# datamicroscopes/common

Measured on AMD Instinct MI355X. Metric: score_value evals/sec, higher is better.
Workload: dtype f32

## Files before the change

common_amd/csrc/kernels_niw.hip:

```cpp
#include <algorithm>
#include <cstdlib>

#include "family_math.hpp"
#include "launchers.hpp"
#include "score_block.hpp"

namespace msc {

typedef float f32x16 __attribute__((ext_vector_type(16)));


MSC_DEV size_t tri(uint32_t i, uint32_t j) { return (size_t)i * (i + 1u) / 2u + j; }
__global__ __launch_bounds__(64) void k_niw_prepare(const FeatDesc *__restrict__ feats, uint32_t f,
                                                     uint32_t K, uint32_t kpad) {
  extern __shared__ __attribute__((aligned(16))) unsigned char smem[];
  const FeatDesc fd = feats[f];
  const uint32_t d = fd.dim, k = blockIdx.x;
  const int t = threadIdx.x;
  const size_t ntri = (size_t)d * (d + 1u) / 2u;
  double *A = reinterpret_cast<double *>(smem);
  double *Li = A + ntri;
  double *mun = Li + ntri;
  double *wmu = mun + d;
  const double kappa = fd.hp[0], nu = fd.hp[1];
// ... 139 lines not shown
  for (uint64_t blk = wave_id; blk < nblocks; blk += nwaves) {
    const uint64_t rb = blk * 32 * T;
    float xr[T][16];
    int gz[T];
    bool live[T], msk[T];
#pragma unroll
    for (int t = 0; t < T; t++) {
      const uint64_t row = rb + 32 * t + r;
      live[t] = row < nrows;
      const float *xp = X + (row0 + (live[t] ? row : 0)) * d + 16 * h;
      if (d == 32) {
#pragma unroll
        for (int q = 0; q < 4; q++) {
          const float4 v = live[t] ? ld4(xp + 4 * q) : make_float4(0, 0, 0, 0);
          xr[t][4 * q] = v.x; xr[t][4 * q + 1] = v.y; xr[t][4 * q + 2] = v.z; xr[t][4 * q + 3] = v.w;
        }
      } else {
#pragma unroll
        for (int s = 0; s < 16; s++) xr[t][s] = (live[t] && (uint32_t)(16 * h + s) < d) ? xp[s] : 0.0f;
      }
      gz[t] = (LOO && live[t]) ? z[row] : -1;
      msk[t] = false;
      if (live[t] && fd.mask != nullptr)
        for (uint32_t e = 0; e < d; e++) msk[t] |= fd.mask[(row0 + row) * d + e] != 0;
    }
    float qkeep[T][4];
    for (uint32_t k = 0; k < K; k++) {
      const float *Wk = fd.niw_w + ((size_t)k * kNiwPad + r) * kNiwPad + 16 * h;
      const float *Bk = fd.niw_b + (size_t)k * 2 * kNiwPad + 16 * h;
      float w[16], mh[16], ml[16];
#pragma unroll
      for (int q = 0; q < 4; q++) {
        const float4 a = ld4(Wk + 4 * q), b = ld4(Bk + 4 * q), c = ld4(Bk + kNiwPad + 4 * q);
        w[4 * q] = a.x; w[4 * q + 1] = a.y; w[4 * q + 2] = a.z; w[4 * q + 3] = a.w;
        mh[4 * q] = b.x; mh[4 * q + 1] = b.y; mh[4 * q + 2] = b.z; mh[4 * q + 3] = b.w;
        ml[4 * q] = c.x; ml[4 * q + 1] = c.y; ml[4 * q + 2] = c.z; ml[4 * q + 3] = c.w;
      }
      const uint32_t slot = k & 3;
      const bool mine = (int)((k >> 2) & 1) == h;
#pragma unroll
      for (int t = 0; t < T; t++) {
        f32x16 acc = {0, 0, 0, 0, 0, 0, 0, 0, 0, 0, 0, 0, 0, 0, 0, 0};
#pragma unroll
        for (int s = 0; s < 16; s++)
          acc = __builtin_amdgcn_mfma_f32_32x32x2f32(w[s], (xr[t][s] - mh[s]) - ml[s], acc, 0, 0, 0);
        float qp = 0.f;
#pragma unroll
        for (int i = 0; i < 16; i++) qp = fmaf(acc[i], acc[i], qp);
        const float q = qp + __shfl_xor(qp, 32, 64);
        if (mine) {
          if (slot == 0) qkeep[t][0] = q;
          else if (slot == 1) qkeep[t][1] = q;
          else if (slot == 2) qkeep[t][2] = q;
          else qkeep[t][3] = q;
        }
      }
      if ((k & 7) == 7 || k == K - 1) {
        const uint32_t k0 = (k & ~7u) + 4 * h;
        float4 pend[T];
#pragma unroll
        for (int i = 0; i < 4; i++) {
          const uint32_t kg = k0 + i;
          const bool valid = kg <= k;
          const size_t kc = valid ? kg : 0;
          const float c0 = fd.tab[(size_t)NIW_C0 * kpad + kc], c1 = fd.tab[(size_t)NIW_C1 * kpad + kc];
#pragma unroll
          for (int t = 0; t < T; t++) {
            const float q = valid ? qkeep[t][i] : 0.f;
            float sc = fmaf(-c1, log1p_acc(q), c0);
            if (LOO && valid && gz[t] == (int)kg) {
              const float y = fminf(fd.tab[(size_t)NIW_C_LOO * kpad + kc] * q, 0.99999994f);
              sc = fmaf(fd.tab[(size_t)NIW_B_LOO * kpad + kc], log1p_acc(-y), fd.tab[(size_t)NIW_A_LOO * kpad + kc]);
            }
            if (msk[t]) sc = 0.f;
            if (i == 0) pend[t].x = sc;
            else if (i == 1) pend[t].y = sc;
            else if (i == 2) pend[t].z = sc;
            else pend[t].w = sc;
          }
        }
#pragma unroll
        for (int t = 0; t < T; t++) {
          if (!live[t] || k0 > k) continue;
          float *p = out + (rb + 32 * t + r) * ld + k0;
          if (vec_ok && k0 + 3 <= k) {
            float4 v = pend[t];
            if (ACCUM) { const float4 o = *reinterpret_cast<const float4 *>(p); v.x += o.x; v.y += o.y; v.z += o.z; v.w += o.w; }
            *reinterpret_cast<float4 *>(p) = v;
          } else {
            const float vals[4] = {pend[t].x, pend[t].y, pend[t].z, pend[t].w};
#pragma unroll
            for (int i = 0; i < 4; i++)
              if (k0 + i <= k) p[i] = ACCUM ? p[i] + vals[i] : vals[i];
          }
        }
      }
    }
  }
}

typedef double f64x4 __attribute__((ext_vector_type(4)));

MSC_DEV double shfl_xor_f64(double v, int mask) {
  const int hi = __shfl_xor(__double2hiint(v), mask, 64), lo = __shfl_xor(__double2loint(v), mask, 64);
  return __hiloint2double(hi, lo);
}

typedef unsigned int u32x2 __attribute__((ext_vector_type(2)));
MSC_DEV double xsum_rows_f64(double v) {
  u32x2 a = __builtin_amdgcn_permlane16_swap((unsigned)__double2loint(v), (unsigned)__double2loint(v), false, false);
  u32x2 b = __builtin_amdgcn_permlane16_swap((unsigned)__double2hiint(v), (unsigned)__double2hiint(v), false, false);
  const double s = __hiloint2double((int)b[0], (int)a[0]) + __hiloint2double((int)b[1], (int)a[1]);
  a = __builtin_amdgcn_permlane32_swap((unsigned)__double2loint(s), (unsigned)__double2loint(s), false, false);
  b = __builtin_amdgcn_permlane32_swap((unsigned)__double2hiint(s), (unsigned)__double2hiint(s), false, false);
  return __hiloint2double((int)b[0], (int)a[0]) + __hiloint2double((int)b[1], (int)a[1]);
}

template <int ROWS>
MSC_DEV double pair_rows_f64(double x, double y) {
  u32x2 lo, hi;
  if (ROWS == 16) {
    lo = __builtin_amdgcn_permlane16_swap((unsigned)__double2loint(x), (unsigned)__double2loint(y), false, false);
    hi = __builtin_amdgcn_permlane16_swap((unsigned)__double2hiint(x), (unsigned)__double2hiint(y), false, false);
  } else {
    lo = __builtin_amdgcn_permlane32_swap((unsigned)__double2loint(x), (unsigned)__double2loint(y), false, false);
    hi = __builtin_amdgcn_permlane32_swap((unsigned)__double2hiint(x), (unsigned)__double2hiint(y), false, false);
  }
  return __hiloint2double((int)hi[0], (int)lo[0]) + __hiloint2double((int)hi[1], (int)lo[1]);
}

MSC_DEV double log_ge1_f64(double u) {
  int hi = __double2hiint(u);
  int e = (hi >> 20) - 1023;
  double m = __hiloint2double((hi & 0x000fffff) | 0x3ff00000, __double2loint(u));
  if (m > 1.4142135623730951) {
    m *= 0.5;
    e += 1;
  }
  const double den = m + 1.0;
  double y = __builtin_amdgcn_rcp(den);
  y = y * fma(-den, y, 2.0);
  y = y * fma(-den, y, 2.0);
  const double sq = (m - 1.0) * y, s2 = sq * sq;
  double p = 1.0 / 15.0;
  p = fma(p, s2, 1.0 / 13.0);
  p = fma(p, s2, 1.0 / 11.0);
  p = fma(p, s2, 1.0 / 9.0);
  p = fma(p, s2, 1.0 / 7.0);
  p = fma(p, s2, 1.0 / 5.0);
  p = fma(p, s2, 1.0 / 3.0);
  p = fma(p, s2, 1.0);
  return fma((double)e, 0.69314718055994530942, 2.0 * sq * p);
}
MSC_DEV double niw_score_from_q(double c0, double c1, double q) { return c0 - c1 * log_ge1_f64(1.0 + q); }

template <int JB, bool LOO, bool ACCUM, bool FULL = false>
MSC_DEV void niw64_finish_batch(const FeatDesc &fd, uint32_t k, int kk, int c, uint64_t rb, const double (&qkeep)[JB][4],
                                const int (&gz)[JB], const bool (&msk)[JB], const bool (&live)[JB],
                                double *__restrict__ qown, float *__restrict__ out, uint64_t ld, bool vec_ok) {
  const uint32_t k0 = (k & ~15u) + 4 * kk;
  float4 pend[JB];
#pragma unroll
  for (int i = 0; i < 4; i++) {
    const uint32_t kg = k0 + i;
    const bool valid = FULL || kg <= k;
    const double *c64 = fd.niw_c64 + (size_t)(valid ? kg : 0) * 8;
    const double c0 = c64[0], c1 = c64[1];
#pragma unroll
    for (int jb = 0; jb < JB; jb++) {
      const double q = valid ? qkeep[jb][i] : 0.0;
      double sc = niw_score_from_q(c0, c1, q);
      if (LOO && valid && gz[jb] == (int)kg) {
        qown[rb + 16 * jb + c] = q;
        sc = 0.0;
      }
      if (msk[jb]) sc = 0.0;
      const float scf = (float)sc;
      if (i == 0) pend[jb].x = scf;
      else if (i == 1) pend[jb].y = scf;
      else if (i == 2) pend[jb].z = scf;
      else pend[jb].w = scf;
    }
  }
#pragma unroll
  for (int jb = 0; jb < JB; jb++) {
    if (!live[jb] || (!FULL && k0 > k)) continue;
    float *p = out + (rb + 16 * jb + c) * ld + k0;
    if (vec_ok && (FULL || k0 + 3 <= k)) {
      float4 v = pend[jb];
      if (ACCUM) { const float4 o = *reinterpret_cast<const float4 *>(p); v.x += o.x; v.y += o.y; v.z += o.z; v.w += o.w; }
      *reinterpret_cast<float4 *>(p) = v;
    } else {
      const float vals[4] = {pend[jb].x, pend[jb].y, pend[jb].z, pend[jb].w};
#pragma unroll
      for (int i = 0; i < 4; i++)
        if (k0 + i <= k) p[i] = ACCUM ? p[i] + vals[i] : vals[i];
    }
  }
}

template <int NB, int JB, bool LOO, bool ACCUM>
__global__ __launch_bounds__(256) void k_score_niw64(const FeatDesc *__restrict__ feats, uint32_t f,
                                                      uint32_t K, uint32_t kpad, uint64_t row0,
                                                      uint64_t nrows, const int32_t *__restrict__ z,
                                                      double *__restrict__ qown, float *__restrict__ out, uint64_t ld) {
  constexpr int NS = 4 * NB;
  constexpr int NCH = NB * (NB + 1) / 2;
  const FeatDesc fd = feats[f];
  const uint32_t d = fd.dim;
  const int lane = threadIdx.x & 63, c = lane & 15, kk = lane >> 4;
  const uint64_t nblocks = (nrows + 16 * JB - 1) / (16 * JB);
  const uint64_t wave_id = (uint64_t)blockIdx.x * 4 + (threadIdx.x >> 6);
  const uint64_t nwaves = (uint64_t)gridDim.x * 4;
  const float *X = reinterpret_cast<const float *>(fd.col);
  const bool vec_ok = ((ld & 3) == 0) && ((reinterpret_cast<uintptr_t>(out) & 15) == 0);
  for (uint64_t blk = wave_id; blk < nblocks; blk += nwaves) {
    const uint64_t rb = blk * 16 * JB;
    float xf[JB][NS];
    int gz[JB];
    bool live[JB], msk[JB];
#pragma unroll
    for (int jb = 0; jb < JB; jb++) {
      const uint64_t row = rb + 16 * jb + c;
      live[jb] = row < nrows;
      const float *xp = X + (row0 + (live[jb] ? row : 0)) * d + kk;
#pragma unroll
      for (int s = 0; s < NS; s++) xf[jb][s] = (live[jb] && (uint32_t)(4 * s + kk) < d) ? xp[4 * s] : 0.0f;
      gz[jb] = (LOO && live[jb]) ? z[row] : -1;
      msk[jb] = false;
      if (live[jb] && fd.mask != nullptr)
        for (uint32_t e = 0; e < d; e++) msk[jb] |= fd.mask[(row0 + row) * d + e] != 0;
    }
    double qkeep[JB][4];
    for (uint32_t k = 0; k < K; k++) {
      const double *Wk = fd.niw_w64 + (size_t)k * (NCH * 256) + lane * 4;
      const double *Bk = fd.niw_mu64 + (size_t)k * (NB * 256) + lane * 4;
      double qp[JB];
#pragma unroll
      for (int jb = 0; jb < JB; jb++) qp[jb] = 0.0;
      constexpr bool PIPE = NB > 2;
      double2 n01 = {0.0, 0.0}, n23 = {0.0, 0.0};
      if (PIPE) {
        n01 = *reinterpret_cast<const double2 *>(Wk);
        n23 = *reinterpret_cast<const double2 *>(Wk + 2);
      }
#pragma unroll
      for (int b = 0; b < NB; b++) {
        const double2 b01 = *reinterpret_cast<const double2 *>(Bk + b * 256), b23 = *reinterpret_cast<const double2 *>(Bk + b * 256 + 2);
        f64x4 acc[JB];
#pragma unroll
        for (int jb = 0; jb < JB; jb++) acc[jb] = f64x4{-b01.x, -b01.y, -b23.x, -b23.y};
#pragma unroll
        for (int s4 = 0; s4 <= b; s4++) {
          constexpr int kLast = NCH - 1;
          const int ch = b * (b + 1) / 2 + s4;
          const double *wc = Wk + ch * 256;
          double2 a01, a23;
          if (PIPE) {
            a01 = n01;
            a23 = n23;
            if (ch < kLast) {
              n01 = *reinterpret_cast<const double2 *>(wc + 256);
              n23 = *reinterpret_cast<const double2 *>(wc + 256 + 2);
            }
          } else {
            a01 = *reinterpret_cast<const double2 *>(wc);
            a23 = *reinterpret_cast<const double2 *>(wc + 2);
          }
          const double a[4] = {a01.x, a01.y, a23.x, a23.y};
#pragma unroll
          for (int e = 0; e < 4; e++) {
#pragma unroll
            for (int jb = 0; jb < JB; jb++) {
              float xv = xf[jb][4 * s4 + e];
              if (NB > 2) asm volatile("" : "+v"(xv));
              acc[jb] = __builtin_amdgcn_mfma_f64_16x16x4f64(a[e], (double)xv, acc[jb], 0, 0, 0);
            }
          }
          if (PIPE) __builtin_amdgcn_sched_barrier(0);
        }
#pragma unroll
        for (int jb = 0; jb < JB; jb++)
#pragma unroll
          for (int i = 0; i < 4; i++) qp[jb] = fma(acc[jb][i], acc[jb][i], qp[jb]);
      }
      const uint32_t slot = k & 3;
      const bool mine = (int)((k >> 2) & 3) == kk;
#pragma unroll
      for (int jb = 0; jb < JB; jb++) {
        const double q = xsum_rows_f64(qp[jb]);
        if (mine) {
          if (slot == 0) qkeep[jb][0] = q;
          else if (slot == 1) qkeep[jb][1] = q;
          else if (slot == 2) qkeep[jb][2] = q;
          else qkeep[jb][3] = q;
        }
      }
      if ((k & 15) == 15 || k == K - 1) {
        const uint32_t k0 = (k & ~15u) + 4 * kk;
        float4 pend[JB];
#pragma unroll
        for (int i = 0; i < 4; i++) {
          const uint32_t kg = k0 + i;
          const bool valid = kg <= k;
          const double *c64 = fd.niw_c64 + (size_t)(valid ? kg : 0) * 8;
          const double c0 = c64[0], c1 = c64[1];
#pragma unroll
          for (int jb = 0; jb < JB; jb++) {
            const double q = valid ? qkeep[jb][i] : 0.0;
            double sc = niw_score_from_q(c0, c1, q);
            if (LOO && valid && gz[jb] == (int)kg) {
              qown[rb + 16 * jb + c] = q;
              sc = 0.0;
            }
            if (msk[jb]) sc = 0.0;
            const float scf = (float)sc;
            if (i == 0) pend[jb].x = scf;
            else if (i == 1) pend[jb].y = scf;
            else if (i == 2) pend[jb].z = scf;
            else pend[jb].w = scf;
          }
        }
#pragma unroll
        for (int jb = 0; jb < JB; jb++) {
          if (!live[jb] || k0 > k) continue;
          float *p = out + (rb + 16 * jb + c) * ld + k0;
          if (vec_ok && k0 + 3 <= k) {
            float4 v = pend[jb];
            if (ACCUM) { const float4 o = *reinterpret_cast<const float4 *>(p); v.x += o.x; v.y += o.y; v.z += o.z; v.w += o.w; }
            *reinterpret_cast<float4 *>(p) = v;
          } else {
            const float vals[4] = {pend[jb].x, pend[jb].y, pend[jb].z, pend[jb].w};
#pragma unroll
            for (int i = 0; i < 4; i++)
              if (k0 + i <= k) p[i] = ACCUM ? p[i] + vals[i] : vals[i];
          }
        }
      }
    }
  }
}

template <int NB, bool LOO, bool ACCUM>
__global__ __launch_bounds__(256, 2) void k_score_niw64_lag(const FeatDesc *__restrict__ feats, uint32_t f,
                                                             uint32_t K, uint32_t kpad, uint64_t row0,
                                                             uint64_t nrows, const int32_t *z,
                                                             double *__restrict__ qown, float *__restrict__ out, uint64_t ld) {
  static_assert(NB == 1 || NB == 2, "dim <= 32");
  constexpr int JB = 4, NS = 4 * NB, NCH = NB * (NB + 1) / 2;
  const FeatDesc fd = feats[f];
  const uint32_t d = fd.dim;
  const int lane = threadIdx.x & 63, c = lane & 15, kk = lane >> 4;
  const uint64_t nblocks = (nrows + 16 * JB - 1) / (16 * JB);
  const uint64_t wave_id = (uint64_t)blockIdx.x * 4 + (threadIdx.x >> 6);
  const uint64_t nwaves = (uint64_t)gridDim.x * 4;
  const float *X = reinterpret_cast<const float *>(fd.col);
  const bool vec_ok = ((ld & 3) == 0) && ((reinterpret_cast<uintptr_t>(out) & 15) == 0);
  typedef uint32_t u32x4v __attribute__((ext_vector_type(4)));
  const __amdgpu_buffer_rsrc_t Wb = __builtin_amdgcn_make_buffer_rsrc(const_cast<double *>(fd.niw_w64), 0, 0x7fffffff, 0x00020000);
  const __amdgpu_buffer_rsrc_t Bb = __builtin_amdgcn_make_buffer_rsrc(const_cast<double *>(fd.niw_mu64), 0, 0x7fffffff, 0x00020000);
  const uint32_t lane_off = lane * 32;
  const uint32_t Kfull = K & ~15u;
  auto group_at = [&](uint32_t t) -> uint32_t {
    const uint32_t g = t < Kfull ? (t & ~15u) + 4 * (t & 3) + ((t >> 2) & 3) : t;
    return g < K ? g : K - 1;
  };
  for (uint64_t blk = wave_id; blk < nblocks; blk += nwaves) {
    const uint64_t rb = blk * 16 * JB;
    float xn[JB][NS];
    int gz[JB];
    bool live[JB], msk[JB];
#pragma unroll
    for (int jb = 0; jb < JB; jb++) {
      const uint64_t row = rb + 16 * jb + c;
      live[jb] = row < nrows;
      const float *xp = X + (row0 + (live[jb] ? row : 0)) * d;
#pragma unroll
      for (int s = 0; s < NS; s++) {
        const bool has = live[jb] && (uint32_t)(4 * s + kk) < d;
        const float v = xp[has ? 4 * s + kk : 0];
        xn[jb][s] = has ? -v : 0.0f;
      }
      gz[jb] = (LOO && live[jb]) ? z[row] : -1;
      msk[jb] = false;
      if (live[jb] && fd.mask != nullptr)
        for (uint32_t e = 0; e < d; e++) msk[jb] |= fd.mask[(row0 + row) * d + e] != 0;
    }
    double qkeep[JB][4];
    double2 w0[2], w1[2], w2[2], m0[2], m1[2];
    auto load2 = [&](double2 (&o)[2], __amdgpu_buffer_rsrc_t buf, uint32_t byte) {
      const u32x4v lo = __builtin_amdgcn_raw_buffer_load_b128(buf, lane_off, byte, 0);
      const u32x4v hi = __builtin_amdgcn_raw_buffer_load_b128(buf, lane_off + 16, byte, 0);
      o[0] = double2{__hiloint2double((int)lo[1], (int)lo[0]), __hiloint2double((int)lo[3], (int)lo[2])};
      o[1] = double2{__hiloint2double((int)hi[1], (int)hi[0]), __hiloint2double((int)hi[3], (int)hi[2])};
    };
    auto chunk = [&](f64x4 (&acc)[JB], const double2 (&w)[2], int s4, const double2 (*m)[2]) {
      const double a[4] = {w[0].x, w[0].y, w[1].x, w[1].y};
#pragma unroll
      for (int e = 0; e < 4; e++)
#pragma unroll
        for (int jb = 0; jb < JB; jb++) {
          const f64x4 from = (m != nullptr && e == 0) ? f64x4{(*m)[0].x, (*m)[0].y, (*m)[1].x, (*m)[1].y} : acc[jb];
          acc[jb] = __builtin_amdgcn_mfma_f64_16x16x4f64(a[e], (double)xn[jb][4 * s4 + e], from, 0, 0, 0);
        }
    };
    auto squares = [](double (&qp)[JB], const f64x4 (&acc)[JB], bool fresh) {
#pragma unroll
      for (int jb = 0; jb < JB; jb++)
#pragma unroll
        for (int i = 0; i < 4; i++) qp[jb] = (fresh && i == 0) ? acc[jb][i] * acc[jb][i] : fma(acc[jb][i], acc[jb][i], qp[jb]);
    };
    f64x4 accA[JB], accB[JB];
    double qp[JB], held[JB], half[JB];
    if constexpr (NB == 2) {
      const uint32_t g0 = group_at(0), g1 = group_at(1);
      load2(w0, Wb, g0 * (NCH * 2048u));
      load2(m0, Bb, g0 * (NB * 2048u));
      load2(w1, Wb, g0 * (NCH * 2048u) + 2048);
      load2(w2, Wb, g0 * (NCH * 2048u) + 4096);
      load2(m1, Bb, g0 * (NB * 2048u) + 2048);
      chunk(accA, w0, 0, &m0);
      load2(w0, Wb, g1 * (NCH * 2048u));
      load2(m0, Bb, g1 * (NB * 2048u));
    } else {
      const uint32_t g0 = group_at(0), g1 = group_at(1), g2 = group_at(2);
      load2(w0, Wb, g0 * 2048u);
      load2(m0, Bb, g0 * 2048u);
      load2(w1, Wb, g1 * 2048u);
      load2(m1, Bb, g1 * 2048u);
      chunk(accA, w0, 0, &m0);
      load2(w0, Wb, g2 * 2048u);
      load2(m0, Bb, g2 * 2048u);
    }
    for (uint32_t t4 = 0; t4 < K; t4 += 4) {
      const bool tail = t4 >= Kfull;
      const bool mine = (int)((t4 >> 2) & 3) == kk;
#pragma unroll
      for (int i = 0; i < 4; i++) {
        if constexpr (NB == 2) {
          const uint32_t gn = group_at(t4 + i + 1), gn2 = group_at(t4 + i + 2);
          chunk(accB, w1, 0, &m1);
          chunk(accB, w2, 1, nullptr);
          squares(qp, accA, true);
          load2(w1, Wb, gn * (NCH * 2048u) + 2048);
          load2(w2, Wb, gn * (NCH * 2048u) + 4096);
          load2(m1, Bb, gn * (NB * 2048u) + 2048);
          __builtin_amdgcn_sched_barrier(0);
          chunk(accA, w0, 0, &m0);
          squares(qp, accB, false);
          load2(w0, Wb, gn2 * (NCH * 2048u));
          load2(m0, Bb, gn2 * (NB * 2048u));
          __builtin_amdgcn_sched_barrier(0);
        } else {
          const uint32_t gn3 = group_at(t4 + i + 3);
          if ((i & 1) == 0) {
            chunk(accB, w1, 0, &m1);
            squares(qp, accA, true);
            load2(w1, Wb, gn3 * 2048u);
            load2(m1, Bb, gn3 * 2048u);
          } else {
            chunk(accA, w0, 0, &m0);
            squares(qp, accB, true);
            load2(w0, Wb, gn3 * 2048u);
            load2(m0, Bb, gn3 * 2048u);
          }
          __builtin_amdgcn_sched_barrier(0);
        }
        if (!tail) {
          if (i == 0 || i == 2) {
#pragma unroll
            for (int jb = 0; jb < JB; jb++) held[jb] = qp[jb];
          } else {
#pragma unroll
            for (int jb = 0; jb < JB; jb++) {
              const double pr = pair_rows_f64<16>(held[jb], qp[jb]);
              if (i == 1) half[jb] = pr;
              else {
                const double q = pair_rows_f64<32>(half[jb], pr);
                qkeep[jb][0] = qkeep[jb][1];
                qkeep[jb][1] = qkeep[jb][2];
                qkeep[jb][2] = qkeep[jb][3];
                qkeep[jb][3] = q;
              }
            }
          }
        } else {
#pragma unroll
          for (int jb = 0; jb < JB; jb++) {
            const double q = xsum_rows_f64(qp[jb]);
            qkeep[jb][i] = mine ? q : qkeep[jb][i];
          }
        }
      }
      const uint32_t kl = t4 + 3 < K ? t4 + 3 : K - 1;
      if ((kl & 15) == 15) niw64_finish_batch<JB, LOO, ACCUM, true>(fd, kl, kk, c, rb, qkeep, gz, msk, live, qown, out, ld, vec_ok);
      else if (kl == K - 1) niw64_finish_batch<JB, LOO, ACCUM>(fd, kl, kk, c, rb, qkeep, gz, msk, live, qown, out, ld, vec_ok);
    }
  }
}

template <int NB, bool LOO, bool ACCUM>
__global__ __launch_bounds__(256, NB <= 5 ? 3 : 2) void k_score_niw64_wide(const FeatDesc *__restrict__ feats, uint32_t f,
                                                           uint32_t K, uint32_t kpad, uint64_t row0,
                                                           uint64_t nrows, const int32_t *z,
                                                           double *__restrict__ qown, float *__restrict__ out, uint64_t ld) {
  static_assert(NB > 2 && NB <= 8, "32 < dim <= 128");
  constexpr int JB = 2, NS = 4 * NB, NCH = NB * (NB + 1) / 2;
  const FeatDesc fd = feats[f];
  const uint32_t d = fd.dim;
  const int lane = threadIdx.x & 63, c = lane & 15, kk = lane >> 4;
  const uint64_t nblocks = (nrows + 16 * JB - 1) / (16 * JB);
  const uint64_t wave_id = (uint64_t)blockIdx.x * 4 + (threadIdx.x >> 6);
  const uint64_t nwaves = (uint64_t)gridDim.x * 4;
  const float *X = reinterpret_cast<const float *>(fd.col);
  const bool vec_ok = ((ld & 3) == 0) && ((reinterpret_cast<uintptr_t>(out) & 15) == 0);
  typedef uint32_t u32x4v __attribute__((ext_vector_type(4)));
  const __amdgpu_buffer_rsrc_t Wb = __builtin_amdgcn_make_buffer_rsrc(const_cast<double *>(fd.niw_w64), 0, 0x7fffffff, 0x00020000);
  const __amdgpu_buffer_rsrc_t Bb = __builtin_amdgcn_make_buffer_rsrc(const_cast<double *>(fd.niw_mu64), 0, 0x7fffffff, 0x00020000);
  const uint32_t lane_off = lane * 32;
  const uint32_t Kfull = K & ~15u;
  auto group_at = [&](uint32_t t) -> uint32_t {
    const uint32_t g = t < Kfull ? (t & ~15u) + 4 * (t & 3) + ((t >> 2) & 3) : t;
    return g < K ? g : K - 1;
  };
  auto load2 = [&](double2 (&o)[2], __amdgpu_buffer_rsrc_t buf, uint32_t byte) {
    const u32x4v lo = __builtin_amdgcn_raw_buffer_load_b128(buf, lane_off, byte, 0);
    const u32x4v hi = __builtin_amdgcn_raw_buffer_load_b128(buf, lane_off + 16, byte, 0);
    o[0] = double2{__hiloint2double((int)lo[1], (int)lo[0]), __hiloint2double((int)lo[3], (int)lo[2])};
    o[1] = double2{__hiloint2double((int)hi[1], (int)hi[0]), __hiloint2double((int)hi[3], (int)hi[2])};
  };
  for (uint64_t blk = wave_id; blk < nblocks; blk += nwaves) {
    const uint64_t rb = blk * 16 * JB;
    float xn[JB][NS];
    int gz[JB];
    bool live[JB], msk[JB];
#pragma unroll
    for (int jb = 0; jb < JB; jb++) {
      const uint64_t row = rb + 16 * jb + c;
      live[jb] = row < nrows;
      const float *xp = X + (row0 + (live[jb] ? row : 0)) * d;
#pragma unroll
      for (int s = 0; s < NS; s++) {
        const bool has = live[jb] && (uint32_t)(4 * s + kk) < d;
        const float v = xp[has ? 4 * s + kk : 0];
        xn[jb][s] = has ? -v : 0.0f;
      }
      gz[jb] = (LOO && live[jb]) ? z[row] : -1;
      msk[jb] = false;
      if (live[jb] && fd.mask != nullptr)
        for (uint32_t e = 0; e < d; e++) msk[jb] |= fd.mask[(row0 + row) * d + e] != 0;
    }
    double qkeep[JB][4], held[JB], half[JB];
    double2 nxt[2];
    load2(nxt, Wb, group_at(0) * (NCH * 2048u));
    const uint32_t Kt = (K + 3u) & ~3u;
    for (uint32_t t = 0; t < Kt; t++) {
      const uint32_t g = group_at(t), gn = group_at(t + 1);
      const int i = (int)(t & 3u);
      const bool tail = t >= Kfull;
      double qp[JB];
#pragma unroll
      for (int jb = 0; jb < JB; jb++) qp[jb] = 0.0;
#pragma unroll
      for (int b = 0; b < NB; b++) {
        double2 m[2];
        load2(m, Bb, g * (NB * 2048u) + b * 2048u);
        const f64x4 mv = {m[0].x, m[0].y, m[1].x, m[1].y};
        f64x4 acc[JB];
#pragma unroll
        for (int s4 = 0; s4 <= b; s4++) {
          constexpr int kLast = NCH - 1;
          const int ch = b * (b + 1) / 2 + s4;
          const double a[4] = {nxt[0].x, nxt[0].y, nxt[1].x, nxt[1].y};
          if (ch < kLast) load2(nxt, Wb, g * (NCH * 2048u) + (ch + 1) * 2048u);
          else load2(nxt, Wb, gn * (NCH * 2048u));
#pragma unroll
          for (int e = 0; e < 4; e++)
#pragma unroll
            for (int jb = 0; jb < JB; jb++) {
              float xv = xn[jb][4 * s4 + e];
              asm volatile("" : "+v"(xv));
              acc[jb] = __builtin_amdgcn_mfma_f64_16x16x4f64(a[e], (double)xv, (s4 == 0 && e == 0) ? mv : acc[jb], 0, 0, 0);
            }
          __builtin_amdgcn_sched_barrier(0);
        }
#pragma unroll
        for (int jb = 0; jb < JB; jb++)
#pragma unroll
          for (int q = 0; q < 4; q++) qp[jb] = fma(acc[jb][q], acc[jb][q], qp[jb]);
      }
      if (!tail) {
        if (i == 0 || i == 2) {
#pragma unroll
          for (int jb = 0; jb < JB; jb++) held[jb] = qp[jb];
        } else {
#pragma unroll
          for (int jb = 0; jb < JB; jb++) {
            const double pr = pair_rows_f64<16>(held[jb], qp[jb]);
            if (i == 1) half[jb] = pr;
            else {
              const double q = pair_rows_f64<32>(half[jb], pr);
              qkeep[jb][0] = qkeep[jb][1];
              qkeep[jb][1] = qkeep[jb][2];
              qkeep[jb][2] = qkeep[jb][3];
              qkeep[jb][3] = q;
            }
          }
        }
      } else {
        const bool mine = (int)((t >> 2) & 3) == kk;
#pragma unroll
        for (int jb = 0; jb < JB; jb++) {
          const double q = xsum_rows_f64(qp[jb]);
          if (mine) {
            if (i == 0) qkeep[jb][0] = q;
            else if (i == 1) qkeep[jb][1] = q;
            else if (i == 2) qkeep[jb][2] = q;
            else qkeep[jb][3] = q;
          }
        }
      }
      if (i == 3) {
        const uint32_t kl = t < K ? t : K - 1;
        if ((kl & 15) == 15) niw64_finish_batch<JB, LOO, ACCUM, true>(fd, kl, kk, c, rb, qkeep, gz, msk, live, qown, out, ld, vec_ok);
        else if (kl == K - 1) niw64_finish_batch<JB, LOO, ACCUM>(fd, kl, kk, c, rb, qkeep, gz, msk, live, qown, out, ld, vec_ok);
      }
    }
  }
}

MSC_DEV double bcast_f64(double v, int lane) {
  return __hiloint2double(__builtin_amdgcn_readlane(__double2hiint(v), lane), __builtin_amdgcn_readlane(__double2loint(v), lane));
}
template <int D>
__global__ __launch_bounds__(256) void k_score_niw_small(const FeatDesc *__restrict__ feats, uint32_t f, uint32_t K,
                                                          uint32_t kpad, uint64_t row0, uint64_t nrows,
                                                          const int32_t *__restrict__ z, double *__restrict__ qown,
                                                          float *__restrict__ out, uint64_t ld, int accum) {
  const FeatDesc fd = feats[f];
  const int lane = threadIdx.x & 63;
  const uint32_t k = blockIdx.y * 64 + lane;
  const bool has_k = k < K;
  const size_t kc = has_k ? k : 0;
  double w[D * (D + 1) / 2], nb[D];
#pragma unroll
  for (int i = 0; i < D; i++) {
#pragma unroll
    for (int j = 0; j <= i; j++) w[i * (i + 1) / 2 + j] = fd.niw_w64[kc * niw_w_stream(D) + niw_w_index(i, j)];
    nb[i] = -fd.niw_mu64[kc * niw_b_stream(D) + niw_b_index(i)];
// ... 78 lines not shown
                                                           uint64_t row0, uint64_t nrows,
                                                           const int32_t *__restrict__ z, uint32_t *__restrict__ scratch) {
  extern __shared__ uint32_t hist[];
  const FeatDesc fd = feats[f];
  const bool lds = K <= kBucketLdsGroups;
  if (lds) {
    for (uint32_t k = threadIdx.x; k < K; k += 256) hist[k] = 0u;
    __syncthreads();
  }
  const uint64_t per = (nrows + gridDim.x - 1) / gridDim.x, lo = (uint64_t)blockIdx.x * per;
  const uint64_t hi = lo + per < nrows ? lo + per : nrows;
  for (uint64_t n = lo + threadIdx.x; n < hi; n += 256)
    if (niw_row_counts(fd, K, row0 + n, z[n])) atomicAdd(lds ? &hist[z[n]] : &scratch[K + 1 + z[n]], 1u);
  if (lds) {
    __syncthreads();
    for (uint32_t k = threadIdx.x; k < K; k += 256)
      if (hist[k]) atomicAdd(&scratch[K + 1 + k], hist[k]);
  }
}
__global__ __launch_bounds__(1024) void k_niw_bucket_scan(uint32_t K, uint32_t *__restrict__ scratch) {
  __shared__ uint32_t part[1024];
  const uint32_t per = (K + 1023) / 1024, lo = threadIdx.x * per, hi = lo + per < K ? lo + per : K;
  uint32_t s = 0;
  for (uint32_t k = lo; k < hi; k++) s += scratch[K + 1 + k];
  part[threadIdx.x] = s;
  __syncthreads();
  for (int off = 1; off < 1024; off <<= 1) {
    const uint32_t v = threadIdx.x >= (uint32_t)off ? part[threadIdx.x - off] : 0u;
    __syncthreads();
    part[threadIdx.x] += v;
    __syncthreads();
  }
  uint32_t run = threadIdx.x ? part[threadIdx.x - 1] : 0u;
  for (uint32_t k = lo; k < hi; k++) {
    const uint32_t c = scratch[K + 1 + k];
    scratch[k] = run;
    scratch[K + 1 + k] = 0u;
    run += c;
  }
  if (threadIdx.x == 1023) scratch[K] = part[1023];
}
__global__ __launch_bounds__(256) void k_niw_bucket_scatter(const FeatDesc *__restrict__ feats, uint32_t f, uint32_t K,
                                                             uint64_t row0, uint64_t nrows,
                                                             const int32_t *__restrict__ z, uint32_t *__restrict__ scratch) {
  extern __shared__ uint32_t sh[];
  const FeatDesc fd = feats[f];
  uint32_t *idx = scratch + 2 * (size_t)K + 1;
  const uint64_t per = (nrows + gridDim.x - 1) / gridDim.x, lo = (uint64_t)blockIdx.x * per;
  const uint64_t hi = lo + per < nrows ? lo + per : nrows;
  if (K > kBucketLdsGroups) {
    for (uint64_t n = lo + threadIdx.x; n < hi; n += 256) {
      const int g = z[n];
      if (niw_row_counts(fd, K, row0 + n, g)) idx[scratch[g] + atomicAdd(&scratch[K + 1 + g], 1u)] = (uint32_t)n;
    }
    return;
  }
  uint32_t *cnt = sh, *base = sh + K;
  for (uint32_t k = threadIdx.x; k < K; k += 256) cnt[k] = 0u;
  __syncthreads();
  for (uint64_t n = lo + threadIdx.x; n < hi; n += 256)
    if (niw_row_counts(fd, K, row0 + n, z[n])) atomicAdd(&cnt[z[n]], 1u);
  __syncthreads();
  for (uint32_t k = threadIdx.x; k < K; k += 256) {
    base[k] = cnt[k] ? scratch[k] + atomicAdd(&scratch[K + 1 + k], cnt[k]) : 0u;
    cnt[k] = 0u;
  }
  __syncthreads();
  for (uint64_t n = lo + threadIdx.x; n < hi; n += 256) {
    const int g = z[n];
    if (niw_row_counts(fd, K, row0 + n, g)) idx[base[g] + atomicAdd(&cnt[g], 1u)] = (uint32_t)n;
  }
}
__global__ __launch_bounds__(256) void k_niw_group_sums(const FeatDesc *__restrict__ feats, uint32_t f, uint32_t K,
                                                         uint64_t row0, const uint32_t *__restrict__ scratch, int sign) {
  __shared__ float xs[4][2][32];
  __shared__ double red[4][17][64];
  const FeatDesc fd = feats[f];
  const uint32_t d = fd.dim, k = blockIdx.x;
  const uint32_t nt = (d + 31u) / 32u, ti = blockIdx.z / nt, tj = blockIdx.z % nt;
  const int lane = threadIdx.x & 63, wave = threadIdx.x >> 6;
  const uint32_t i = (uint32_t)lane >> 1, half = (uint32_t)lane & 1u;
  const uint32_t beg = scratch[k], end = scratch[k + 1];
  const uint32_t *idx = scratch + 2 * (size_t)K + 1;
  const float *X = reinterpret_cast<const float *>(fd.col);
  double sxx[16], sx = 0.0;
#pragma unroll
  for (int j = 0; j < 16; j++) sxx[j] = 0.0;
  for (uint32_t p = beg + blockIdx.y * 4 + wave; p < end; p += gridDim.y * 4) {
    const float *x = X + (row0 + idx[p]) * d;
    const uint32_t e = (uint32_t)(lane & 31), src = 32u * (lane < 32 ? ti : tj) + e;
    xs[wave][lane >> 5][e] = src < d ? x[src] : 0.f;
    const double xi = (double)xs[wave][0][i];
    if (half == 0) sx += xi;
#pragma unroll
    for (int j = 0; j < 16; j++) sxx[j] = fma(xi, (double)xs[wave][1][half * 16 + j], sxx[j]);
  }
#pragma unroll
  for (int j = 0; j < 16; j++) red[wave][j][lane] = sxx[j];
  red[wave][16][lane] = sx;
  __syncthreads();
  if (end == beg) return;
  const size_t stride = d + (size_t)d * d;
  double *dst = fd.acc_f64 + (size_t)k * stride;
  for (uint32_t e = threadIdx.x; e < 17 * 64; e += 256) {
    const uint32_t j = e >> 6, l = e & 63, ii = 32u * ti + (l >> 1), hh = l & 1u;
    const double v = red[0][j][l] + red[1][j][l] + red[2][j][l] + red[3][j][l];
    if (ii >= d) continue;
    if (j == 16) {
      if (tj == 0 && hh == 0 && v != 0.0) atomicAdd(&dst[ii], (double)sign * v);
    } else {
      const uint32_t col = 32u * tj + hh * 16 + j;
      if (col < d && v != 0.0) atomicAdd(&dst[d + (size_t)ii * d + col], (double)sign * v);
    }
  }
  if (blockIdx.y == 0 && blockIdx.z == 0 && threadIdx.x == 0)
    atomicAdd(reinterpret_cast<unsigned long long *>(&fd.acc_i64[k]), (unsigned long long)((long long)sign * (long long)(end - beg)));
}

__global__ __launch_bounds__(256) void k_niw_commit(const FeatDesc *__restrict__ feats, uint32_t f,
                                                     uint32_t K, uint32_t kpad, int to_raw) {
  const FeatDesc fd = feats[f];
  const size_t stride = fd.dim + (size_t)fd.dim * fd.dim, total = (size_t)K * stride;
  const size_t i = (size_t)blockIdx.x * 256 + threadIdx.x;
  if (i < total) {
    if (to_raw) fd.raw_f32[i] = (float)fd.acc_f64[i];
    else fd.acc_f64[i] = (double)fd.raw_f32[i];
  }
  if (i < kpad) {
    if (to_raw) fd.raw_u32[i] = (uint32_t)fd.acc_i64[i];
    else fd.acc_i64[i] = fd.raw_u32[i];
  }
}

int launch_niw_prepare(hipStream_t stream, const FeatDesc *feats_dev, uint32_t f, uint32_t dim, uint32_t K,
                       uint32_t kpad) {
  const size_t lds = sizeof(double) * ((size_t)dim * (dim + 1) + 2 * (size_t)dim);
  static unsigned long long attr_devices = 0;
  if (lds > 64u * 1024u && first_use_on_device(attr_devices))
    (void)hipFuncSetAttribute(reinterpret_cast<const void *>(k_niw_prepare), hipFuncAttributeMaxDynamicSharedMemorySize, 160 * 1024);
  hipLaunchKernelGGL(k_niw_prepare, dim3(K + 1), dim3(64), lds, stream, feats_dev, f, K, kpad);
  return hipGetLastError() == hipSuccess ? 0 : -1;
}

int launch_niw_score_data(hipStream_t stream, const FeatDesc *feats_dev, uint32_t f, uint32_t K,
                          uint32_t kpad, float *out) {
  hipLaunchKernelGGL(k_niw_score_data, dim3((K + 255) / 256), dim3(256), 0, stream, feats_dev, f, K, kpad, out);
  return hipGetLastError() == hipSuccess ? 0 : -1;
}

template <int NB, bool LOO, bool ACCUM>
static void launch_niw64_nb(hipStream_t stream, const dim3 grid, const FeatDesc *feats_dev, uint32_t f, uint32_t K, uint32_t kpad,
                            uint64_t row0, uint64_t nrows, const int32_t *z, double *qown, float *out, uint64_t ld) {
  if constexpr (NB <= 2) {
    if ((uint64_t)K * 6144u < 0x7fffffffull) {
      hipLaunchKernelGGL((k_score_niw64_lag<NB, LOO, ACCUM>), (note_kernel(0, "k_score_niw64_lag<%d, %s, %s>", NB, tf(LOO), tf(ACCUM)), grid), dim3(256), 0, stream, feats_dev, f, K, kpad, row0, nrows, z, qown, out, ld);
      return;
    }
  }
  if constexpr (NB > 2) {
    if ((uint64_t)K * (NB * (NB + 1) / 2) * 2048u < 0x7fffffffull)
      hipLaunchKernelGGL((k_score_niw64_wide<NB, LOO, ACCUM>), (note_kernel(0, "k_score_niw64_wide<%d, %s, %s>", NB, tf(LOO), tf(ACCUM)), dim3(grid.x * 2)), dim3(256), 0, stream, feats_dev, f, K, kpad, row0, nrows, z, qown, out, ld);
    else
      hipLaunchKernelGGL((k_score_niw64<NB, 2, LOO, ACCUM>), (note_kernel(0, "k_score_niw64<%d, 2, %s, %s>", NB, tf(LOO), tf(ACCUM)), dim3(grid.x * 2)), dim3(256), 0, stream, feats_dev, f, K, kpad, row0, nrows, z, qown, out, ld);
  } else
    hipLaunchKernelGGL((k_score_niw64<NB, 4, LOO, ACCUM>), (note_kernel(0, "k_score_niw64<%d, 4, %s, %s>", NB, tf(LOO), tf(ACCUM)), grid), dim3(256), 0, stream, feats_dev, f, K, kpad, row0, nrows, z, qown, out, ld);
}
template <bool LOO, bool ACCUM>
static void launch_niw_score_t(hipStream_t stream, int num_cus, bool f32_fast, uint32_t dim, const FeatDesc *feats_dev,
                               uint32_t f, uint32_t K, uint32_t kpad, uint64_t row0, uint64_t nrows,
                               const int32_t *z, double *qown, float *out, uint64_t ld) {
  constexpr int kRowsPerWave = 64;
  const uint64_t nblocks = (nrows + kRowsPerWave - 1) / kRowsPerWave;
  uint64_t gx = (nblocks + 3) / 4;
  const uint64_t cap = (uint64_t)num_cus * 8;
  if (gx > cap) gx = cap;
  const dim3 grid((unsigned)(gx ? gx : 1)), block(256);
  if (f32_fast && dim <= (uint32_t)kNiwPad)
    hipLaunchKernelGGL((k_score_niw<2, LOO, ACCUM>), (note_kernel(0, "k_score_niw<2, %s, %s>", tf(LOO), tf(ACCUM)), grid), block, 0, stream, feats_dev, f, K, kpad, row0, nrows, z, out, ld);
  else {
    switch (niw_blocks(dim)) {
      case 1: launch_niw64_nb<1, LOO, ACCUM>(stream, grid, feats_dev, f, K, kpad, row0, nrows, z, qown, out, ld); break;
      case 2: launch_niw64_nb<2, LOO, ACCUM>(stream, grid, feats_dev, f, K, kpad, row0, nrows, z, qown, out, ld); break;
      case 3: launch_niw64_nb<3, LOO, ACCUM>(stream, grid, feats_dev, f, K, kpad, row0, nrows, z, qown, out, ld); break;
      case 4: launch_niw64_nb<4, LOO, ACCUM>(stream, grid, feats_dev, f, K, kpad, row0, nrows, z, qown, out, ld); break;
      case 5: launch_niw64_nb<5, LOO, ACCUM>(stream, grid, feats_dev, f, K, kpad, row0, nrows, z, qown, out, ld); break;
      case 6: launch_niw64_nb<6, LOO, ACCUM>(stream, grid, feats_dev, f, K, kpad, row0, nrows, z, qown, out, ld); break;
      case 7: launch_niw64_nb<7, LOO, ACCUM>(stream, grid, feats_dev, f, K, kpad, row0, nrows, z, qown, out, ld); break;
      default: launch_niw64_nb<8, LOO, ACCUM>(stream, grid, feats_dev, f, K, kpad, row0, nrows, z, qown, out, ld); break;
    }
    if (LOO)
      hipLaunchKernelGGL(k_niw_loo_patch, dim3((unsigned)((nrows + 255) / 256)), dim3(256), 0, stream, feats_dev, f, K, row0,
                         nrows, z, qown, out, ld);
  }
}

template <int D>
static void launch_niw_small(hipStream_t stream, int num_cus, const FeatDesc *feats_dev, uint32_t f, uint32_t K, uint32_t kpad,
                             uint64_t row0, uint64_t nrows, const int32_t *z, double *qown, float *out, uint64_t ld, bool accum) {
  const uint32_t ktiles = (K + 63) / 64;
  uint64_t gx = ((nrows + 63) / 64 + 3) / 4;
  const uint64_t cap = std::max<uint64_t>(1, (uint64_t)num_cus * 8 / ktiles);
  if (gx > cap) gx = cap;
  hipLaunchKernelGGL(k_score_niw_small<D>, dim3((unsigned)(gx ? gx : 1), ktiles), dim3(256), 0, stream, feats_dev, f, K, kpad,
                     row0, nrows, z, qown, out, ld, accum ? 1 : 0);
  if (z != nullptr)
    hipLaunchKernelGGL(k_niw_loo_patch, dim3((unsigned)((nrows + 255) / 256)), dim3(256), 0, stream, feats_dev, f, K, row0,
                       nrows, z, qown, out, ld);
}

int launch_niw_score(hipStream_t stream, int num_cus, const FeatDesc *feats_dev, uint32_t f, uint32_t dim, uint32_t K,
                     uint32_t kpad, uint64_t row0, uint64_t nrows, const int32_t *z, bool accum, bool f32_fast,
                     double *qown, float *out, uint64_t ld) {
  if (!f32_fast && dim >= 1 && dim <= 8 && nrows > 0) {
    switch (dim) {
      case 1: launch_niw_small<1>(stream, num_cus, feats_dev, f, K, kpad, row0, nrows, z, qown, out, ld, accum); break;
      case 2: launch_niw_small<2>(stream, num_cus, feats_dev, f, K, kpad, row0, nrows, z, qown, out, ld, accum); break;
      case 3: launch_niw_small<3>(stream, num_cus, feats_dev, f, K, kpad, row0, nrows, z, qown, out, ld, accum); break;
      case 4: launch_niw_small<4>(stream, num_cus, feats_dev, f, K, kpad, row0, nrows, z, qown, out, ld, accum); break;
      case 5: launch_niw_small<5>(stream, num_cus, feats_dev, f, K, kpad, row0, nrows, z, qown, out, ld, accum); break;
      case 6: launch_niw_small<6>(stream, num_cus, feats_dev, f, K, kpad, row0, nrows, z, qown, out, ld, accum); break;
      case 7: launch_niw_small<7>(stream, num_cus, feats_dev, f, K, kpad, row0, nrows, z, qown, out, ld, accum); break;
      default: launch_niw_small<8>(stream, num_cus, feats_dev, f, K, kpad, row0, nrows, z, qown, out, ld, accum); break;
    }
    return hipGetLastError() == hipSuccess ? 0 : -1;
  }
  if (z && accum) launch_niw_score_t<true, true>(stream, num_cus, f32_fast, dim, feats_dev, f, K, kpad, row0, nrows, z, qown, out, ld);
  else if (z) launch_niw_score_t<true, false>(stream, num_cus, f32_fast, dim, feats_dev, f, K, kpad, row0, nrows, z, qown, out, ld);
  else if (accum) launch_niw_score_t<false, true>(stream, num_cus, f32_fast, dim, feats_dev, f, K, kpad, row0, nrows, z, qown, out, ld);
  else launch_niw_score_t<false, false>(stream, num_cus, f32_fast, dim, feats_dev, f, K, kpad, row0, nrows, z, qown, out, ld);
  return hipGetLastError() == hipSuccess ? 0 : -1;
}

template <int D>
__global__ __launch_bounds__(1024) void k_niw_accumulate_small(const FeatDesc *__restrict__ feats, uint32_t f, uint32_t K,
                                                                uint64_t row0, uint64_t nrows, const int32_t *__restrict__ z,
                                                                int sign) {
  extern __shared__ __attribute__((aligned(16))) unsigned char smem[];
  constexpr uint32_t kStride = D + D * D;
  const FeatDesc fd = feats[f];
  double *sums = reinterpret_cast<double *>(smem);
  uint32_t *cnt = reinterpret_cast<uint32_t *>(sums + (size_t)K * kStride);
  for (uint32_t i = threadIdx.x; i < K * kStride; i += blockDim.x) sums[i] = 0.0;
  for (uint32_t i = threadIdx.x; i < K; i += blockDim.x) cnt[i] = 0u;
  __syncthreads();
  const uint64_t per = (nrows + gridDim.x - 1) / gridDim.x;
  const uint64_t lo = (uint64_t)blockIdx.x * per, hi = lo + per < nrows ? lo + per : nrows;
  const float *X = reinterpret_cast<const float *>(fd.col);
  for (uint64_t n = lo + threadIdx.x; n < hi; n += blockDim.x) {
    const int g = z[n];
    const uint64_t row = row0 + n;
    if (!niw_row_counts(fd, K, row, g)) continue;
    double x[D];
#pragma unroll
    for (int j = 0; j < D; j++) x[j] = (double)X[row * D + j];
    double *dst = sums + (size_t)g * kStride;
    atomicAdd(&cnt[g], 1u);
#pragma unroll
    for (int i = 0; i < D; i++) {
      atomicAdd(&dst[i], x[i]);
#pragma unroll
      for (int j = 0; j < D; j++) atomicAdd(&dst[D + i * D + j], x[i] * x[j]);
    }
  }
  __syncthreads();
  for (uint32_t i = threadIdx.x; i < K * kStride; i += blockDim.x)
    if (sums[i] != 0.0) atomicAdd(&fd.acc_f64[i], (double)sign * sums[i]);
  for (uint32_t i = threadIdx.x; i < K; i += blockDim.x)
    if (cnt[i]) atomicAdd(reinterpret_cast<unsigned long long *>(&fd.acc_i64[i]), (unsigned long long)((long long)sign * (long long)cnt[i]));
}
template <int D>
static void launch_niw_accumulate_small(hipStream_t stream, int num_cus, const FeatDesc *feats_dev, uint32_t f, uint32_t K,
                                        uint64_t row0, uint64_t nrows, const int32_t *z, int sign, size_t lds) {
  static unsigned long long attr_devices = 0;
  if (first_use_on_device(attr_devices))
    (void)hipFuncSetAttribute(reinterpret_cast<const void *>(k_niw_accumulate_small<D>),
                              hipFuncAttributeMaxDynamicSharedMemorySize, 160 * 1024);
  uint64_t blocks = (nrows + 4095) / 4096;
  if (blocks < (uint64_t)num_cus) blocks = (nrows + 1023) / 1024;
  if (blocks > (uint64_t)num_cus * 2) blocks = (uint64_t)num_cus * 2;
  hipLaunchKernelGGL(k_niw_accumulate_small<D>, dim3((unsigned)(blocks ? blocks : 1)), dim3(1024), lds, stream, feats_dev, f, K,
                     row0, nrows, z, sign);
}

int launch_niw_accumulate(hipStream_t stream, int num_cus, const FeatDesc *feats_dev, uint32_t f, uint32_t K,
                          uint64_t row0, uint64_t nrows, const int32_t *z, int sign, uint32_t *scratch_dev, uint32_t dim) {
  if (nrows == 0) return 0;
  const size_t small_lds = (size_t)K * ((dim + (size_t)dim * dim) * sizeof(double) + sizeof(uint32_t));
  if (dim >= 1 && dim <= 8 && small_lds <= 96u * 1024u) {
    switch (dim) {
      case 1: launch_niw_accumulate_small<1>(stream, num_cus, feats_dev, f, K, row0, nrows, z, sign, small_lds); break;
      case 2: launch_niw_accumulate_small<2>(stream, num_cus, feats_dev, f, K, row0, nrows, z, sign, small_lds); break;
      case 3: launch_niw_accumulate_small<3>(stream, num_cus, feats_dev, f, K, row0, nrows, z, sign, small_lds); break;
      case 4: launch_niw_accumulate_small<4>(stream, num_cus, feats_dev, f, K, row0, nrows, z, sign, small_lds); break;
      case 5: launch_niw_accumulate_small<5>(stream, num_cus, feats_dev, f, K, row0, nrows, z, sign, small_lds); break;
      case 6: launch_niw_accumulate_small<6>(stream, num_cus, feats_dev, f, K, row0, nrows, z, sign, small_lds); break;
      case 7: launch_niw_accumulate_small<7>(stream, num_cus, feats_dev, f, K, row0, nrows, z, sign, small_lds); break;
      default: launch_niw_accumulate_small<8>(stream, num_cus, feats_dev, f, K, row0, nrows, z, sign, small_lds); break;
    }
    return hipGetLastError() == hipSuccess ? 0 : -1;
  }
  if (hipMemsetAsync(scratch_dev, 0, sizeof(uint32_t) * (2 * (size_t)K + 1), stream) != hipSuccess) return -1;
  uint64_t gx = (nrows + 255) / 256;
  const uint64_t cap = (uint64_t)num_cus * 8;
  if (gx > cap) gx = cap;
  const size_t lds1 = K <= kBucketLdsGroups ? sizeof(uint32_t) * K : 0, lds2 = 2 * lds1;
  hipLaunchKernelGGL(k_niw_bucket_count, dim3((unsigned)gx), dim3(256), lds1, stream, feats_dev, f, K, row0, nrows, z, scratch_dev);
  hipLaunchKernelGGL(k_niw_bucket_scan, dim3(1), dim3(1024), 0, stream, K, scratch_dev);
// ... 21 lines not shown
```

Measured before the change: 1478 billion.

## Finish NIW scores per group inside lag kernel loop with buffer stores

Restructures the lagged NIW64 scoring kernel so each 4-cluster group's score is computed and written immediately after its reduction, rather than keeping a shifting qkeep buffer and calling a batched finish routine every 16 clusters. Score constants and outputs go through buffer resources, and the log coefficients are pinned in scalar registers. Inputs are widened to double once at load time rather than inside each MFMA. This cuts register pressure and spreads the transcendental and store work across the MFMA pipeline, at the cost of more, smaller scalar stores. A new launch guard keeps 32-bit buffer offsets valid.

Result: no change. 1473 billion, median of 6 (-0.3%).

```diff
diff --git a/common_amd/csrc/kernels_niw.hip b/common_amd/csrc/kernels_niw.hip
--- a/common_amd/csrc/kernels_niw.hip
+++ b/common_amd/csrc/kernels_niw.hip
@@ -315,7 +315,35 @@
   p = fma(p, s2, 1.0);
   return fma((double)e, 0.69314718055994530942, 2.0 * sq * p);
 }
+#define MSC_LOG_GE1_COEFS \
+  {1.0 / 15.0, 1.0 / 13.0, 1.0 / 11.0, 1.0 / 9.0, 1.0 / 7.0, 1.0 / 5.0, 1.0 / 3.0, 1.4142135623730951, 0.69314718055994530942}
+MSC_DEV double log_ge1_f64(double u, const double (&k)[9], int bias) {
+  int hi = __double2hiint(u);
+  int e = (hi >> 20) - bias;
+  double m = __hiloint2double((hi & 0x000fffff) | 0x3ff00000, __double2loint(u));
+  if (m > k[7]) {
+    m *= 0.5;
+    e += 1;
+  }
+  const double den = m + 1.0;
+  double y = __builtin_amdgcn_rcp(den);
+  y = y * fma(-den, y, 2.0);
+  y = y * fma(-den, y, 2.0);
+  const double sq = (m - 1.0) * y, s2 = sq * sq;
+  double p = k[0];
+  p = fma(p, s2, k[1]);
+  p = fma(p, s2, k[2]);
+  p = fma(p, s2, k[3]);
+  p = fma(p, s2, k[4]);
+  p = fma(p, s2, k[5]);
+  p = fma(p, s2, k[6]);
+  p = fma(p, s2, 1.0);
+  return fma((double)e, k[8], 2.0 * sq * p);
+}
 MSC_DEV double niw_score_from_q(double c0, double c1, double q) { return c0 - c1 * log_ge1_f64(1.0 + q); }
+MSC_DEV double niw_score_from_q(double c0, double c1, double q, const double (&k)[9], int bias) {
+  return c0 - c1 * log_ge1_f64(1.0 + q, k, bias);
+}
 
 template <int JB, bool LOO, bool ACCUM, bool FULL = false>
 MSC_DEV void niw64_finish_batch(const FeatDesc &fd, uint32_t k, int kk, int c, uint64_t rb, const double (&qkeep)[JB][4],
@@ -518,11 +546,12 @@
   const uint64_t wave_id = (uint64_t)blockIdx.x * 4 + (threadIdx.x >> 6);
   const uint64_t nwaves = (uint64_t)gridDim.x * 4;
   const float *X = reinterpret_cast<const float *>(fd.col);
-  const bool vec_ok = ((ld & 3) == 0) && ((reinterpret_cast<uintptr_t>(out) & 15) == 0);
   typedef uint32_t u32x4v __attribute__((ext_vector_type(4)));
   const __amdgpu_buffer_rsrc_t Wb = __builtin_amdgcn_make_buffer_rsrc(const_cast<double *>(fd.niw_w64), 0, 0x7fffffff, 0x00020000);
   const __amdgpu_buffer_rsrc_t Bb = __builtin_amdgcn_make_buffer_rsrc(const_cast<double *>(fd.niw_mu64), 0, 0x7fffffff, 0x00020000);
+  const __amdgpu_buffer_rsrc_t Cb = __builtin_amdgcn_make_buffer_rsrc(fd.niw_c64, 0, 0x7fffffff, 0x00020000);
   const uint32_t lane_off = lane * 32;
+  const uint32_t row_off = (uint32_t)c * (uint32_t)ld * 4u + 16u * kk;
   const uint32_t Kfull = K & ~15u;
   auto group_at = [&](uint32_t t) -> uint32_t {
     const uint32_t g = t < Kfull ? (t & ~15u) + 4 * (t & 3) + ((t >> 2) & 3) : t;
@@ -530,26 +559,32 @@
   };
   for (uint64_t blk = wave_id; blk < nblocks; blk += nwaves) {
     const uint64_t rb = blk * 16 * JB;
-    float xn[JB][NS];
+    const __amdgpu_buffer_rsrc_t Ob = __builtin_amdgcn_make_buffer_rsrc(out + rb * ld, 0, 0x7fffffff, 0x00020000);
+    const __amdgpu_buffer_rsrc_t Qb = __builtin_amdgcn_make_buffer_rsrc(LOO ? qown + rb : qown, 0, 0x7fffffff, 0x00020000);
+    double xn[JB][NS];
     int gz[JB];
     bool live[JB], msk[JB];
+    uint32_t cr = (uint32_t)c;
+    asm volatile("" : "+v"(cr));
 #pragma unroll
     for (int jb = 0; jb < JB; jb++) {
-      const uint64_t row = rb + 16 * jb + c;
+      const uint64_t row = rb + 16 * jb + cr;
       live[jb] = row < nrows;
-      const float *xp = X + (row0 + (live[jb] ? row : 0)) * d;
-#pragma unroll
-      for (int s = 0; s < NS; s++) {
-        const bool has = live[jb] && (uint32_t)(4 * s + kk) < d;
-        const float v = xp[has ? 4 * s + kk : 0];
-        xn[jb][s] = has ? -v : 0.0f;
-      }
       gz[jb] = (LOO && live[jb]) ? z[row] : -1;
       msk[jb] = false;
       if (live[jb] && fd.mask != nullptr)
         for (uint32_t e = 0; e < d; e++) msk[jb] |= fd.mask[(row0 + row) * d + e] != 0;
     }
-    double qkeep[JB][4];
+#pragma unroll
+    for (int jb = 0; jb < JB; jb++) {
+      const float *xp = X + (row0 + (live[jb] ? rb + 16 * jb + cr : 0)) * d;
+#pragma unroll
+      for (int s = 0; s < NS; s++) {
+        const bool has = live[jb] && (uint32_t)(4 * s + kk) < d;
+        const float v = xp[has ? 4 * s + kk : 0];
+        xn[jb][s] = has ? -(double)v : 0.0;
+      }
+    }
     double2 w0[2], w1[2], w2[2], m0[2], m1[2];
     auto load2 = [&](double2 (&o)[2], __amdgpu_buffer_rsrc_t buf, uint32_t byte) {
       const u32x4v lo = __builtin_amdgcn_raw_buffer_load_b128(buf, lane_off, byte, 0);
@@ -564,7 +599,7 @@
 #pragma unroll
         for (int jb = 0; jb < JB; jb++) {
           const f64x4 from = (m != nullptr && e == 0) ? f64x4{(*m)[0].x, (*m)[0].y, (*m)[1].x, (*m)[1].y} : acc[jb];
-          acc[jb] = __builtin_amdgcn_mfma_f64_16x16x4f64(a[e], (double)xn[jb][4 * s4 + e], from, 0, 0, 0);
+          acc[jb] = __builtin_amdgcn_mfma_f64_16x16x4f64(a[e], xn[jb][4 * s4 + e], from, 0, 0, 0);
         }
     };
     auto squares = [](double (&qp)[JB], const f64x4 (&acc)[JB], bool fresh) {
@@ -574,7 +609,62 @@
         for (int i = 0; i < 4; i++) qp[jb] = (fresh && i == 0) ? acc[jb][i] * acc[jb][i] : fma(acc[jb][i], acc[jb][i], qp[jb]);
     };
     f64x4 accA[JB], accB[JB];
-    double qp[JB], held[JB], half[JB];
+    double qp[JB];
+    auto step = [&](uint32_t t, int i) {
+      if constexpr (NB == 2) {
+        const uint32_t gn = group_at(t + 1), gn2 = group_at(t + 2);
+        chunk(accB, w1, 0, &m1);
+        chunk(accB, w2, 1, nullptr);
+        squares(qp, accA, true);
+        load2(w1, Wb, gn * (NCH * 2048u) + 2048);
+        load2(w2, Wb, gn * (NCH * 2048u) + 4096);
+        load2(m1, Bb, gn * (NB * 2048u) + 2048);
+        __builtin_amdgcn_sched_barrier(0);
+        chunk(accA, w0, 0, &m0);
+        squares(qp, accB, false);
+        load2(w0, Wb, gn2 * (NCH * 2048u));
+        load2(m0, Bb, gn2 * (NB * 2048u));
+        __builtin_amdgcn_sched_barrier(0);
+      } else {
+        const uint32_t gn3 = group_at(t + 3);
+        if ((i & 1) == 0) {
+          chunk(accB, w1, 0, &m1);
+          squares(qp, accA, true);
+          load2(w1, Wb, gn3 * 2048u);
+          load2(m1, Bb, gn3 * 2048u);
+        } else {
+          chunk(accA, w0, 0, &m0);
+          squares(qp, accB, true);
+          load2(w0, Wb, gn3 * 2048u);
+          load2(m0, Bb, gn3 * 2048u);
+        }
+        __builtin_amdgcn_sched_barrier(0);
+      }
+    };
+    auto file = [&](uint32_t kg, bool take, const u32x4v cw, const double (&q)[JB], uint32_t voff, uint32_t soff) {
+      const double c0 = __hiloint2double((int)cw[1], (int)cw[0]), c1 = __hiloint2double((int)cw[3], (int)cw[2]);
+      double lk[9] = MSC_LOG_GE1_COEFS;
+      int bias = 1023;
+#pragma unroll
+      for (int i = 0; i < 9; i++) asm volatile("" : "+s"(lk[i]));
+      asm volatile("" : "+s"(bias));
+#pragma unroll
+      for (int jb = 0; jb < JB; jb++) {
+        double sc = niw_score_from_q(c0, c1, q[jb], lk, bias);
+        if (LOO && take && gz[jb] == (int)kg) {
+          const u32x2 qw = {(uint32_t)__double2loint(q[jb]), (uint32_t)__double2hiint(q[jb])};
+          __builtin_amdgcn_raw_buffer_store_b64(qw, Qb, (uint32_t)c * 8u, 128u * jb, 0);
+          sc = 0.0;
+        }
+        if (msk[jb]) sc = 0.0;
+        float v = (float)sc;
+        if (take && live[jb]) {
+          const uint32_t so = 16u * jb * (uint32_t)ld * 4u + soff;
+          if (ACCUM) v += __uint_as_float(__builtin_amdgcn_raw_buffer_load_b32(Ob, voff, so, 0));
+          __builtin_amdgcn_raw_buffer_store_b32(__float_as_uint(v), Ob, voff, so, 0);
+        }
+      }
+    };
     if constexpr (NB == 2) {
       const uint32_t g0 = group_at(0), g1 = group_at(1);
       load2(w0, Wb, g0 * (NCH * 2048u));
@@ -595,69 +685,37 @@
       load2(w0, Wb, g2 * 2048u);
       load2(m0, Bb, g2 * 2048u);
     }
-    for (uint32_t t4 = 0; t4 < K; t4 += 4) {
-      const bool tail = t4 >= Kfull;
+    for (uint32_t b16 = 0; b16 < Kfull; b16 += 16) {
+#pragma unroll
+      for (int s = 0; s < 4; s++) {
+        const uint32_t kg = b16 + 4 * kk + s;
+        const u32x4v cw = __builtin_amdgcn_raw_buffer_load_b128(Cb, 256u * kk, (b16 + s) * 64u, 0);
+        double held[JB], half[JB];
+#pragma unroll
+        for (int i = 0; i < 4; i++) {
+          step(b16 + 4 * s + i, i);
+#pragma unroll
+          for (int jb = 0; jb < JB; jb++) {
+            if (i == 0 || i == 2) held[jb] = qp[jb];
+            else if (i == 1) half[jb] = pair_rows_f64<16>(held[jb], qp[jb]);
+            else qp[jb] = pair_rows_f64<32>(half[jb], pair_rows_f64<16>(held[jb], qp[jb]));
+          }
+        }
+        file(kg, true, cw, qp, row_off, (b16 + s) * 4u);
+      }
+    }
+    for (uint32_t t4 = Kfull; t4 < K; t4 += 4) {
       const bool mine = (int)((t4 >> 2) & 3) == kk;
 #pragma unroll
       for (int i = 0; i < 4; i++) {
-        if constexpr (NB == 2) {
-          const uint32_t gn = group_at(t4 + i + 1), gn2 = group_at(t4 + i + 2);
-          chunk(accB, w1, 0, &m1);
-          chunk(accB, w2, 1, nullptr);
-          squares(qp, accA, true);
-          load2(w1, Wb, gn * (NCH * 2048u) + 2048);
-          load2(w2, Wb, gn * (NCH * 2048u) + 4096);
-          load2(m1, Bb, gn * (NB * 2048u) + 2048);
-          __builtin_amdgcn_sched_barrier(0);
-          chunk(accA, w0, 0, &m0);
-          squares(qp, accB, false);
-          load2(w0, Wb, gn2 * (NCH * 2048u));
-          load2(m0, Bb, gn2 * (NB * 2048u));
-          __builtin_amdgcn_sched_barrier(0);
-        } else {
-          const uint32_t gn3 = group_at(t4 + i + 3);
-          if ((i & 1) == 0) {
-            chunk(accB, w1, 0, &m1);
-            squares(qp, accA, true);
-            load2(w1, Wb, gn3 * 2048u);
-            load2(m1, Bb, gn3 * 2048u);
-          } else {
-            chunk(accA, w0, 0, &m0);
-            squares(qp, accB, true);
-            load2(w0, Wb, gn3 * 2048u);
-            load2(m0, Bb, gn3 * 2048u);
-          }
-          __builtin_amdgcn_sched_barrier(0);
-        }
-        if (!tail) {
-          if (i == 0 || i == 2) {
-#pragma unroll
-            for (int jb = 0; jb < JB; jb++) held[jb] = qp[jb];
-          } else {
-#pragma unroll
-            for (int jb = 0; jb < JB; jb++) {
-              const double pr = pair_rows_f64<16>(held[jb], qp[jb]);
-              if (i == 1) half[jb] = pr;
-              else {
-                const double q = pair_rows_f64<32>(half[jb], pr);
-                qkeep[jb][0] = qkeep[jb][1];
-                qkeep[jb][1] = qkeep[jb][2];
-                qkeep[jb][2] = qkeep[jb][3];
-                qkeep[jb][3] = q;
-              }
-            }
-          }
-        } else {
-#pragma unroll
-          for (int jb = 0; jb < JB; jb++) {
-            const double q = xsum_rows_f64(qp[jb]);
-            qkeep[jb][i] = mine ? q : qkeep[jb][i];
-          }
-        }
-      }
-      const uint32_t kl = t4 + 3 < K ? t4 + 3 : K - 1;
-      if ((kl & 15) == 15) niw64_finish_batch<JB, LOO, ACCUM, true>(fd, kl, kk, c, rb, qkeep, gz, msk, live, qown, out, ld, vec_ok);
-      else if (kl == K - 1) niw64_finish_batch<JB, LOO, ACCUM>(fd, kl, kk, c, rb, qkeep, gz, msk, live, qown, out, ld, vec_ok);
+        step(t4 + i, i);
+        const uint32_t kg = t4 + i;
+        const bool take = mine && kg < K;
+        const u32x4v cw = __builtin_amdgcn_raw_buffer_load_b128(Cb, take ? kg * 64u : 0u, 0, 0);
+#pragma unroll
+        for (int jb = 0; jb < JB; jb++) qp[jb] = xsum_rows_f64(qp[jb]);
+        file(kg, take, cw, qp, (uint32_t)c * (uint32_t)ld * 4u + kg * 4u, 0);
+      }
     }
   }
 }
@@ -1042,7 +1100,7 @@
 static void launch_niw64_nb(hipStream_t stream, const dim3 grid, const FeatDesc *feats_dev, uint32_t f, uint32_t K, uint32_t kpad,
                             uint64_t row0, uint64_t nrows, const int32_t *z, double *qown, float *out, uint64_t ld) {
   if constexpr (NB <= 2) {
-    if ((uint64_t)K * 6144u < 0x7fffffffull) {
+    if ((uint64_t)K * 6144u < 0x7fffffffull && (uint64_t)64 * ld * 4u + (uint64_t)K * 4u < 0x7fffffffull) {
       hipLaunchKernelGGL((k_score_niw64_lag<NB, LOO, ACCUM>), (note_kernel(0, "k_score_niw64_lag<%d, %s, %s>", NB, tf(LOO), tf(ACCUM)), grid), dim3(256), 0, stream, feats_dev, f, K, kpad, row0, nrows, z, qown, out, ld);
       return;
     }
```
